# AIGC-Audio/AudioGPT

Hardware: AMD Instinct MI355X
Metric: generated audio-seconds/sec (10s clip, 100 DDIM steps) [3 independent batches of 8 prompts in flight per GPU] (higher is better)
Workload: dtype bf16x3; 1 GPU; Make-An-Audio T2A batch=8/GPU, 100 DDIM steps, CFG 1.5, UNet+VAE+HiFi-GAN(16k), fp32 storage, bf16x3-split MFMA (hi/lo, fp32 accumulate; meets the fp32 parity gates); prompts_per_gpu=8, ddim_steps=100, mel_frames=624, hipgraph=True, batches_in_flight=3, cfg_lanes=1, concurrency_hint=3, parallelism=prompt-sharded x1 (RCCL bcast cond / gather wav)

## Files before the change

### audiogpt_amd/_lib.py

```python
import ctypes as C
import os

import torch

_HERE = os.path.dirname(os.path.abspath(__file__))
LIB_PATH = os.environ.get("AUDIOGPT_AMD_LIB") or os.path.join(_HERE, "libaudiogpt_mi355x.so")


class MaaError(RuntimeError):
    pass


class maa_tensor(C.Structure):
    _fields_ = [("name", C.c_char_p), ("data", C.POINTER(C.c_float)), ("ndim", C.c_int), ("shape", C.c_int64 * 6)]


class maa_prof_row(C.Structure):
    _fields_ = [("name", C.c_char * 48), ("launches", C.c_int64), ("ms", C.c_double), ("flops", C.c_double),
                ("bytes", C.c_double)]


class maa_unet_config(C.Structure):
    _fields_ = [("in_channels", C.c_int), ("out_channels", C.c_int), ("model_channels", C.c_int),
                ("num_res_blocks", C.c_int),
# ... 22 lines not shown
                ("embed_dim", C.c_int), ("resolution", C.c_int), ("num_res_blocks", C.c_int), ("double_z", C.c_int),
                ("n_ch_mult", C.c_int), ("ch_mult", C.c_int * 8),
                ("n_attn_resolutions", C.c_int), ("attn_resolutions", C.c_int * 8)]


class maa_vocoder_config(C.Structure):
    _fields_ = [("kind", C.c_int), ("num_mels", C.c_int), ("upsample_initial_channel", C.c_int),
                ("n_upsamples", C.c_int), ("upsample_rates", C.c_int * 8), ("upsample_kernel_sizes", C.c_int * 8),
                ("n_kernels", C.c_int), ("resblock_kernel_sizes", C.c_int * 8),
                ("n_dilations", C.c_int), ("resblock_dilation_sizes", (C.c_int * 8) * 8),
                ("snake_beta", C.c_int), ("snake_logscale", C.c_int),
                ("use_pitch_embed", C.c_int), ("sampling_rate", C.c_int), ("harmonic_num", C.c_int),
                ("resblock", C.c_int)]


class maa_diffnet_config(C.Structure):
    _fields_ = [("in_dims", C.c_int), ("hidden_size", C.c_int), ("residual_layers", C.c_int),
                ("residual_channels", C.c_int), ("dilation_cycle_length", C.c_int)]


class maa_encoder_config(C.Structure):
    _fields_ = [("kind", C.c_int), ("layers", C.c_int), ("width", C.c_int), ("heads", C.c_int), ("mlp_dim", C.c_int),
                ("d_proj", C.c_int), ("vocab", C.c_int), ("max_positions", C.c_int), ("patch", C.c_int),
                ("image", C.c_int), ("ln_eps", C.c_float)]


class maa_clap_audio_config(C.Structure):
    _fields_ = [("mel_bins", C.c_int), ("n_blocks", C.c_int), ("channels", C.c_int * 8), ("out_emb", C.c_int),
                ("d_proj", C.c_int), ("bn_eps", C.c_float)]


class maa_spectral_config(C.Structure):
    _fields_ = [("n_fft", C.c_int), ("hop", C.c_int), ("n_freq", C.c_int), ("n_mels", C.c_int), ("pad_mode", C.c_int),
                ("power", C.c_int), ("log_kind", C.c_int), ("amin", C.c_float), ("ref", C.c_float), ("out_layout", C.c_int)]


class maa_plms_args(C.Structure):
    _fields_ = [("B", C.c_int), ("T", C.c_int), ("K_step", C.c_int), ("interval", C.c_int), ("timesteps", C.c_int),
                ("d_cond", C.c_void_p), ("h_alphas_cumprod", C.POINTER(C.c_float)), ("use_graph", C.c_int)]


EXPORTS = [
    "maa_last_error", "maa_version", "maa_ctx_create", "maa_ctx_destroy", "maa_ctx_synchronize",
    "maa_ctx_set_stream", "maa_ctx_set_precision", "maa_ctx_set_cfg_split", "maa_ctx_set_concurrency", "maa_ctx_reload_tuning", "maa_ctx_workspace_bytes", "maa_prof_begin", "maa_prof_end", "maa_unet_create", "maa_unet_destroy",
    "maa_unet_set_context", "maa_unet_forward", "maa_ddim_update", "maa_ddim_sample", "maa_ddim_stochastic_encode", "maa_ddim_decode",
    "maa_ldm_plms_sample",
    "maa_vae_create",
    "maa_vae_destroy", "maa_vae_decode", "maa_vae_decode_spec", "maa_vae_encode_moments", "maa_vocoder_create", "maa_vocoder_destroy",
    "maa_vocoder_forward", "maa_vocoder_forward_f0", "maa_diffnet_create", "maa_diffnet_destroy", "maa_diffnet_forward",
    "maa_plms_sample", "maa_encoder_create", "maa_encoder_destroy", "maa_encoder_text", "maa_encoder_image",
    "maa_encoder_text_cls", "maa_clap_audio_create", "maa_clap_audio_destroy", "maa_clap_audio_embed", "maa_clap_similarity",
    "maa_spectral_create", "maa_spectral_destroy", "maa_spectral_forward", "maa_resampler_create", "maa_resampler_destroy",
    "maa_resampler_forward", "maa_op_linear", "maa_op_conv", "maa_op_groupnorm", "maa_op_layernorm",
    "maa_op_attention", "maa_op_conv_transpose1d", "maa_op_snake_aa", "maa_op_bench_conv", "maa_calib",
]

_lib = None


def load():
    global _lib
    if _lib is not None:
        return _lib
    if not os.path.exists(LIB_PATH):
        raise MaaError("%s not found -- run `python -m audiogpt_amd.build` (hipcc, gfx950)" % LIB_PATH)
    try:
        lib = C.CDLL(LIB_PATH)
    except OSError as e:
        raise MaaError("cannot load %s: %s" % (LIB_PATH, e))
    vp, ci, cf, fp = C.c_void_p, C.c_int, C.c_float, C.POINTER(C.c_float)
    lib.maa_last_error.restype = C.c_char_p
    lib.maa_version.restype = C.c_char_p
    sig = {
        "maa_ctx_create": [ci, vp, C.POINTER(vp)],
        "maa_ctx_destroy": [vp],
        "maa_ctx_synchronize": [vp],
        "maa_ctx_set_stream": [vp, vp],
        "maa_ctx_workspace_bytes": [vp, C.POINTER(C.c_size_t)],
        "maa_ctx_set_precision": [vp, ci],
        "maa_ctx_set_cfg_split": [vp, ci],
        "maa_ctx_set_concurrency": [vp, ci],
        "maa_ctx_reload_tuning": [vp],
        "maa_prof_begin": [vp, ci],
        "maa_prof_end": [vp, C.POINTER(maa_prof_row), ci, C.POINTER(ci)],
        "maa_unet_create": [vp, C.POINTER(maa_unet_config), C.POINTER(maa_tensor), ci, C.POINTER(vp)],
        "maa_unet_destroy": [vp],
        "maa_unet_set_context": [vp, vp, vp, ci, ci],
        "maa_unet_forward": [vp, vp, vp, vp, ci, ci, ci, vp],
        "maa_ddim_update": [vp, vp, vp, vp, cf, vp, C.c_int64, vp, vp],
        "maa_ddim_sample": [vp, vp, C.POINTER(maa_ddim_args), vp],
        "maa_ddim_stochastic_encode": [vp, vp, ci, cf, vp, vp, fp, fp, ci, vp, ci, ci, ci, ci, vp],
        "maa_ddim_decode": [vp, vp, C.POINTER(maa_ddim_args), ci, vp],
        "maa_ldm_plms_sample": [vp, vp, C.POINTER(maa_ddim_args), vp],
        "maa_vae_create": [vp, C.POINTER(maa_vae_config), C.POINTER(maa_tensor), ci, C.POINTER(vp)],
        "maa_vae_destroy": [vp],
        "maa_vae_decode": [vp, vp, vp, ci, ci, ci, cf, vp],
        "maa_vae_decode_spec": [vp, vp, vp, ci, ci, ci, cf, vp],
        "maa_vae_encode_moments": [vp, vp, vp, ci, ci, ci, vp],
        "maa_vocoder_create": [vp, C.POINTER(maa_vocoder_config), C.POINTER(maa_tensor), ci, C.POINTER(vp)],
        "maa_vocoder_destroy": [vp],
        "maa_vocoder_forward": [vp, vp, vp, ci, ci, vp],
        "maa_vocoder_forward_f0": [vp, vp, vp, vp, vp, vp, ci, ci, vp],
        "maa_diffnet_create": [vp, C.POINTER(maa_diffnet_config), C.POINTER(maa_tensor), ci, C.POINTER(vp)],
        "maa_diffnet_destroy": [vp],
        "maa_diffnet_forward": [vp, vp, vp, vp, vp, ci, ci, vp],
        "maa_plms_sample": [vp, vp, C.POINTER(maa_plms_args), vp],
        "maa_encoder_create": [vp, C.POINTER(maa_encoder_config), C.POINTER(maa_tensor), ci, C.POINTER(vp)],
        "maa_encoder_destroy": [vp],
        "maa_encoder_text": [vp, vp, vp, ci, ci, vp],
        "maa_encoder_image": [vp, vp, vp, ci, vp],
        "maa_encoder_text_cls": [vp, vp, vp, ci, ci, vp],
        "maa_clap_audio_create": [vp, C.POINTER(maa_clap_audio_config), C.POINTER(maa_tensor), ci, C.POINTER(vp)],
        "maa_clap_audio_destroy": [vp],
        "maa_clap_audio_embed": [vp, vp, vp, ci, ci, vp, vp],
        "maa_clap_similarity": [vp, vp, vp, ci, ci, ci, cf, vp],
        "maa_spectral_create": [vp, C.POINTER(maa_spectral_config), fp, fp, C.POINTER(vp)],
        "maa_spectral_destroy": [vp],
        "maa_spectral_forward": [vp, vp, vp, ci, ci, vp],
        "maa_resampler_create": [vp, ci, ci, ci, ci, fp, C.POINTER(vp)],
        "maa_resampler_destroy": [vp],
        "maa_resampler_forward": [vp, vp, vp, ci, ci, vp],
        "maa_op_linear": [vp, vp, ci, ci, fp, fp, ci, ci, vp],
        "maa_op_conv": [vp, vp, ci, ci, ci, ci, fp, fp, ci, ci, ci, ci, ci, ci, ci, cf, vp, ci, ci],
        "maa_op_groupnorm": [vp, vp, ci, ci, ci, fp, fp, cf, ci, vp],
        "maa_op_layernorm": [vp, vp, ci, ci, fp, fp, cf, vp],
        "maa_op_attention": [vp, vp, vp, vp, ci, ci, ci, ci, ci, cf, vp],
        "maa_op_conv_transpose1d": [vp, vp, ci, ci, ci, fp, fp, ci, ci, ci, cf, vp],
        "maa_op_snake_aa": [vp, vp, ci, ci, ci, fp, fp, ci, vp],
        "maa_op_bench_conv": [vp, ci, ci, ci, ci, ci, ci, ci, ci, C.POINTER(C.c_float)],
        "maa_calib": [vp, ci, C.POINTER(C.c_double)],
    }
    for name, argtypes in sig.items():
        fn = getattr(lib, name)
        fn.argtypes = argtypes
        fn.restype = ci
    _lib = lib
    return lib


def check(status):
    if status != 0:
        raise MaaError("libaudiogpt_mi355x: %s (status %d)" % (load().maa_last_error().decode(), status))


def host_f32(t):
    t = t.detach().to(device="cpu", dtype=torch.float32).contiguous()
    return t, C.cast(t.data_ptr(), C.POINTER(C.c_float))


def tensor_list(state_dict):
    items = list(state_dict.items())
    arr = (maa_tensor * len(items))()
    keep = []
    for i, (name, t) in enumerate(items):
        ht, ptr = host_f32(t)
        bname = name.encode()
        keep.append((ht, bname))
        arr[i].name = bname
        arr[i].data = ptr
        arr[i].ndim = ht.dim()
        for d, s in enumerate(ht.shape):
            arr[i].shape[d] = s
    return arr, len(items), keep


def dptr(t):
    assert t.is_cuda and t.dtype == torch.float32 and t.is_contiguous(), (t.device, t.dtype, t.is_contiguous())
    return C.c_void_p(t.data_ptr())
```

### audiogpt_amd/backend.py

```python
import ctypes as C
import threading
import weakref

import numpy as np
import torch

from . import _lib as L


def default_precision():
    import os
    p = os.environ.get("AUDIOGPT_AMD_PRECISION", "bf16x3")
    if p not in Context.PRECISIONS:
        raise ValueError("AUDIOGPT_AMD_PRECISION must be one of %s" % sorted(Context.PRECISIONS))
    return p


_contexts = weakref.WeakSet()


def reload_tuning():
    for c in list(_contexts):
        c.reload_tuning()

# ... 73 lines not shown
    def __del__(self):
        try:
            self.close()
        except Exception:
            pass

    def op_linear(self, a, w, b=None, geglu=False):
        a = _f32(a, self.device)
        M, K = a.shape
        N = w.shape[0]
        wt, wp = L.host_f32(w)
        bt, bp = L.host_f32(b) if b is not None else (None, None)
        y = torch.empty(M, N // 2 if geglu else N, device=self.device)
        L.check(self.lib.maa_op_linear(self.h, L.dptr(a), M, K, wp, bp, N, int(geglu), L.dptr(y)))
        return y

    def op_conv(self, x, w, b=None, stride=1, pad=0, dil=1, up=False, leaky=0.0, out_hw=None):
        x = _f32(x, self.device)
        B, Cin, H, W = x.shape
        Cout, _, KH, KW = w.shape
        if out_hw is None:
            He, We = (2 * H, 2 * W) if up else (H, W)
            ph = pad if KH > 1 else 0
            Ho = (He + 2 * ph - dil * (KH - 1) - 1) // stride + 1
            Wo = (We + 2 * pad - dil * (KW - 1) - 1) // stride + 1
        else:
            Ho, Wo = out_hw
        wt, wp = L.host_f32(w)
        bt, bp = L.host_f32(b) if b is not None else (None, None)
        y = torch.empty(B, Cout, Ho, Wo, device=self.device)
        L.check(self.lib.maa_op_conv(self.h, L.dptr(x), B, Cin, H, W, wp, bp, Cout, KH, KW, stride, pad, dil,
                                     int(up), float(leaky), L.dptr(y), Ho, Wo))
        return y

    def op_groupnorm(self, x, gamma, beta, eps, silu=False):
        x = _f32(x, self.device)
        B, Cc = x.shape[:2]
        HW = int(np.prod(x.shape[2:]))
        gt, gp = L.host_f32(gamma)
        bt, bp = L.host_f32(beta)
        y = torch.empty_like(x)
        L.check(self.lib.maa_op_groupnorm(self.h, L.dptr(x), B, Cc, HW, gp, bp, float(eps), int(silu), L.dptr(y)))
        return y

    def op_layernorm(self, x, gamma, beta, eps=1e-5):
        x = _f32(x, self.device)
        rows, Cc = x.reshape(-1, x.shape[-1]).shape
        gt, gp = L.host_f32(gamma)
        bt, bp = L.host_f32(beta)
        y = torch.empty_like(x)
        L.check(self.lib.maa_op_layernorm(self.h, L.dptr(x), rows, Cc, gp, bp, float(eps), L.dptr(y)))
        return y

    def op_attention(self, q, k, v, heads, alpha):
        q, k, v = _f32(q, self.device), _f32(k, self.device), _f32(v, self.device)
        B, Nq, Cc = q.shape
        Nk = k.shape[1]
        y = torch.empty_like(q)
        L.check(self.lib.maa_op_attention(self.h, L.dptr(q), L.dptr(k), L.dptr(v), B, heads, Cc // heads, Nq, Nk,
                                          float(alpha), L.dptr(y)))
        return y

    def op_conv_transpose1d(self, x, w, b, stride, leaky=0.0):
        x = _f32(x, self.device)
        B, Cin, Ln = x.shape
        _, Cout, k = w.shape
        wt, wp = L.host_f32(w)
        bt, bp = L.host_f32(b)
        y = torch.empty(B, Cout, Ln * stride, device=self.device)
        L.check(self.lib.maa_op_conv_transpose1d(self.h, L.dptr(x), B, Cin, Ln, wp, bp, Cout, k, stride, float(leaky),
                                                 L.dptr(y)))
        return y

    def op_bench_conv(self, B, H, W, Cin, Cout, taps=9, pre_split=True, iters=20):
        ms = C.c_float()
        L.check(self.lib.maa_op_bench_conv(self.h, B, H, W, Cin, Cout, taps, int(pre_split), iters, C.byref(ms)))
        return ms.value

    def op_snake_aa(self, x, alpha, beta, logscale):
        x = _f32(x, self.device)
        B, Cc, Ln = x.shape
        at, ap = L.host_f32(alpha)
        bt, bp = L.host_f32(beta)
        y = torch.empty_like(x)
        L.check(self.lib.maa_op_snake_aa(self.h, L.dptr(x), B, Cc, Ln, ap, bp, int(logscale), L.dptr(y)))
        return y


def _fill(arr, values):
    for i, v in enumerate(values):
        arr[i] = int(v)
    return len(values)


class UNet:

    def __init__(self, ctx, cfg, state_dict):
        self.ctx, self.cfg = ctx, cfg
        c = L.maa_unet_config()
        c.in_channels, c.out_channels, c.model_channels = cfg["in_channels"], cfg["out_channels"], cfg["model_channels"]
        c.num_res_blocks = cfg["num_res_blocks"]
        c.n_channel_mult = _fill(c.channel_mult, cfg["channel_mult"])
        c.n_attention_resolutions = _fill(c.attention_resolutions, cfg["attention_resolutions"])
        c.num_heads, c.num_head_channels = cfg["num_heads"], cfg["num_head_channels"]
        c.use_spatial_transformer = int(cfg["use_spatial_transformer"])
        c.transformer_depth = cfg.get("transformer_depth", 1)
        c.context_dim = cfg["context_dim"] or 0
        c.legacy, c.resblock_updown = int(cfg["legacy"]), int(cfg["resblock_updown"])
        c.add_context_to_emb = int(cfg.get("add_context_to_emb", False))
        arr, n, keep = L.tensor_list(state_dict)
        h = C.c_void_p()
        with ctx.lock:
            L.check(ctx.lib.maa_unet_create(ctx.h, C.byref(c), arr, n, C.byref(h)))
# ... 625 lines not shown
```

### audiogpt_amd/csrc/api.cpp

```cpp
#include "models.h"

#include <cstring>
#include <memory>

namespace maa {
const char* last_error_cstr();
}

struct maa_ctx {
    maa::Ctx c;
    bool owns_stream = false;
};
struct maa_unet {
    std::unique_ptr<maa::UNet> m;
};
struct maa_vae {
    std::unique_ptr<maa::VAE> m;
};
struct maa_vocoder {
    std::unique_ptr<maa::Vocoder> m;
};
struct maa_diffnet {
    std::unique_ptr<maa::DiffNet> m;
};
// ... 605 lines not shown
    });
}

int maa_calib(maa_ctx* ctx, int kind, double* out_value) {
    return guarded([&] {
        bind(ctx);
        MAA_CHECK(out_value && kind >= 0 && kind <= 3, "bad calib arguments");
        *out_value = maa::calib_run(ctx->c, kind);
    });
}

int maa_op_groupnorm(maa_ctx* ctx, const float* d_x, int B, int C, int HW, const float* h_gamma, const float* h_beta,
                     float eps, int silu, float* d_y) {
    return guarded([&] {
        bind(ctx);
        MAA_CHECK(d_x && h_gamma && h_beta && d_y, "bad op_groupnorm arguments");
        maa::WeightStore ws(ctx->c.dtype != 0);
        maa::Ctx& c = ctx->c;
        float* g = ws.upload(std::vector<float>(h_gamma, h_gamma + C));
        float* b = ws.upload(std::vector<float>(h_beta, h_beta + C));
        maa::run_sized(c, [&] {
            maa::T4 x = maa::alloc_t(c, B, 1, HW, C), y = maa::alloc_t(c, B, 1, HW, C);
            maa::launch_nchw_to_nhwc(c, d_x, B, C, HW, x.p);
            maa::launch_groupnorm(c, x.p, C, C, nullptr, 0, 0, B, HW, 32, g, b, eps, silu, y.p);
            maa::launch_nhwc_to_nchw(c, y.p, B, C, HW, d_y, C);
        });
        MAA_HIP(hipStreamSynchronize(c.stream));
    });
}

int maa_op_layernorm(maa_ctx* ctx, const float* d_x, int rows, int C, const float* h_gamma, const float* h_beta,
                     float eps, float* d_y) {
    return guarded([&] {
        bind(ctx);
        MAA_CHECK(d_x && h_gamma && h_beta && d_y, "bad op_layernorm arguments");
        maa::WeightStore ws(ctx->c.dtype != 0);
        maa::Ctx& c = ctx->c;
        float* g = ws.upload(std::vector<float>(h_gamma, h_gamma + C));
        float* b = ws.upload(std::vector<float>(h_beta, h_beta + C));
        maa::launch_layernorm(c, d_x, rows, C, g, b, eps, d_y);
        MAA_HIP(hipStreamSynchronize(c.stream));
    });
}

int maa_op_attention(maa_ctx* ctx, const float* d_q, const float* d_k, const float* d_v, int B, int heads, int dh,
                     int Nq, int Nk, float alpha, float* d_y) {
    return guarded([&] {
        bind(ctx);
        MAA_CHECK(d_q && d_k && d_v && d_y, "bad op_attention arguments");
        maa::Ctx& c = ctx->c;
        const int C = heads * dh;
        maa::run_sized(c, [&] {
            maa::attention_into(c, d_q, C, dh, d_k, C, dh, d_v, C, dh, B, heads, dh, Nq, Nk, alpha, d_y, C);
        });
        MAA_HIP(hipStreamSynchronize(c.stream));
    });
}

int maa_op_conv_transpose1d(maa_ctx* ctx, const float* d_x, int B, int Cin, int L, const float* h_w,
                            const float* h_bias, int Cout, int k, int stride, float leaky_slope, float* d_y) {
    return guarded([&] {
        bind(ctx);
        MAA_CHECK(d_x && h_w && h_bias && d_y, "bad op_conv_transpose1d arguments");
        OneShot s;
        s.add("w", h_w, {Cin, Cout, k});
        s.add("b", h_bias, {Cout});
        maa::WeightStore ws(ctx->c.dtype != 0);
        maa::Ctx& c = ctx->c;
        const int pad = (k - stride) / 2, U = k / stride;
        maa::run_sized(c, [&] {
            maa::T4 x = maa::alloc_t(c, B, 1, L, Cin), y = maa::alloc_t(c, B, 1, L * stride, Cout);
            maa::launch_nchw_to_nhwc(c, d_x, B, Cin, L, x.p);
            for (int carry = 0; carry < 2; ++carry) {
                bool any = false;
                for (int r = 0; r < stride; ++r) any = any || ((r + pad) / stride == carry);
                if (!any) continue;
                int r_start = 0, r_count = 0;
                maa::PackedW pw;
                if (!c.ws.dry) pw = ws.pack_convtr_phase(s.sd, "w", "b", stride, pad, carry, &r_start, &r_count);
                maa::IGemm p;
                p.a1 = x.p;
                p.lda1 = Cin;
                p.C1 = Cin;
                p.Win = L;
                p.Wout = L;
                p.KW = U;
                p.pw = U - 1 - carry;
                if (leaky_slope != 0.f) {
                    p.a_act = 1;
                    p.a_slope = leaky_slope;
                }
                p.b = pw.w;
                p.ldb = pw.ld;
                p.b_nk = pw.nk;
                p.b_split = pw.split;
                p.M = B * L;
                p.K = U * Cin;
                p.N = r_count * Cout;
                p.bias = pw.bias;
                p.c = y.p + (long long)r_start * Cout;
                p.ldc = stride * Cout;
                if (!c.ws.dry) maa::launch_igemm(c, p);
            }
            maa::launch_nhwc_to_nchw(c, y.p, B, Cout, L * stride, d_y, Cout);
        });
        MAA_HIP(hipStreamSynchronize(c.stream));
// ... 114 lines not shown
```

### audiogpt_amd/csrc/flash_attn.hip

```cpp
#include "maa_internal.h"

#include <cstdlib>

namespace maa {

typedef float f32x16 __attribute__((ext_vector_type(16)));
typedef __bf16 bf16x8 __attribute__((ext_vector_type(8)));
typedef __bf16 bf16x2 __attribute__((ext_vector_type(2)));
typedef float f32x2 __attribute__((ext_vector_type(2)));

struct FlashArgs {
    const float *q, *k, *v;
    int ldq, ldk, ldv;
    int hsq, hsk, hsv;
    long long q_bs, k_bs, v_bs;
    int heads, Nq, Nk;
    float scale;
    float* out;
    int ldo;
    int out_split;
    int causal;
    int qtiles, xcd_on;
    long long o_bs;
    const float* zeros;
};

namespace {

constexpr int NT = 256;
constexpr int KT = 32;

__device__ __forceinline__ unsigned pk_bf16(float a, float b) {
    f32x2 f = {a, b};
    bf16x2 h = __builtin_convertvector(f, bf16x2);
    return __builtin_bit_cast(unsigned, h);
}
__device__ __forceinline__ void split2(float a, float b, unsigned& hi, unsigned& lo) {
    hi = pk_bf16(a, b);
    lo = pk_bf16(a - __builtin_bit_cast(float, hi << 16), b - __builtin_bit_cast(float, hi & 0xffff0000u));
}
struct Frag {
    unsigned w[4];
};
__device__ __forceinline__ bf16x8 as_bf16x8(const Frag& f) { return __builtin_bit_cast(bf16x8, f); }

template <int DH, int TERMS>
__global__ __launch_bounds__(NT, 1) void flash_attn_kernel(const FlashArgs a) {
    constexpr int DK = (DH + 15) / 16 * 16;
    constexpr int DM = (DH + 31) / 32 * 32;
    constexpr int KS = DK / 16, MB = DM / 32;
    constexpr int PL = TERMS == 1 ? 1 : 2;
    constexpr int LDKK = DK + 8;
    constexpr int LDV = KT + 4;
    constexpr int K_PLANE = KT * LDKK, V_PLANE = DM * LDV;
    constexpr int BUF = PL * (K_PLANE + V_PLANE);
    constexpr int C4 = DH / 4;
    static_assert(DH % 8 == 0, "head dim");
    extern __shared__ __attribute__((aligned(16))) unsigned short smem[];

    const int tid = threadIdx.x, lane = tid & 63, wid = tid >> 6;
    const int lq = lane & 31, lh = lane >> 5;
    const int w = xcd_contiguous((int)blockIdx.x, (int)gridDim.x, a.xcd_on);
    const int bh = w / a.qtiles, b = bh / a.heads, h = bh - b * a.heads;
    const int q0 = (w - bh * a.qtiles) * 128 + wid * 32;
    const bool wave_live = q0 < a.Nq;
    const float* qp = a.q + b * a.q_bs + h * a.hsq;
    const float* kp = a.k + b * a.k_bs + h * a.hsk;
    const float* vp = a.v + b * a.v_bs + h * a.hsv;
    const float4* zero4 = reinterpret_cast<const float4*>(a.zeros);

    for (int i = tid; i < 2 * BUF / 2; i += NT) reinterpret_cast<unsigned*>(smem)[i] = 0u;

    Frag qh[KS], ql[KS];
    {
        const int qrow = q0 + lq;
        const bool qok = qrow < a.Nq;
        const float* src = qp + (long long)(qok ? qrow : 0) * a.ldq;
        const float qs = a.scale * 1.4426950408889634f;
#pragma unroll
        for (int ks = 0; ks < KS; ++ks) {
            const int d = ks * 16 + lh * 8;
            float4 x0 = *((qok && d < DH) ? reinterpret_cast<const float4*>(src + d) : zero4);
            float4 x1 = *((qok && d + 4 < DH) ? reinterpret_cast<const float4*>(src + d + 4) : zero4);
            x0.x *= qs;
            x0.y *= qs;
            x0.z *= qs;
            x0.w *= qs;
            x1.x *= qs;
            x1.y *= qs;
            x1.z *= qs;
            x1.w *= qs;
            if constexpr (TERMS == 1) {
                qh[ks].w[0] = pk_bf16(x0.x, x0.y);
                qh[ks].w[1] = pk_bf16(x0.z, x0.w);
                qh[ks].w[2] = pk_bf16(x1.x, x1.y);
                qh[ks].w[3] = pk_bf16(x1.z, x1.w);
            } else {
                split2(x0.x, x0.y, qh[ks].w[0], ql[ks].w[0]);
                split2(x0.z, x0.w, qh[ks].w[1], ql[ks].w[1]);
                split2(x1.x, x1.y, qh[ks].w[2], ql[ks].w[2]);
                split2(x1.z, x1.w, qh[ks].w[3], ql[ks].w[3]);
            }
        }
    }

    constexpr int C2 = DH / 2;
    constexpr int NK = KT * C4, NV = (KT / 4) * C2;
    constexpr int NLK = (NK + NT - 1) / NT, NLV = (NV + NT - 1) / NT;
    float4 rk[NLK];
    float2 rv[NLV][4];
    const float2* zero2 = reinterpret_cast<const float2*>(a.zeros);
    auto load_tile = [&](int kt) {
#pragma unroll
        for (int j = 0; j < NLK; ++j) {
            const int idx = tid + NT * j;
            const int key = idx / C4, c4 = idx - key * C4;
            const int kg = kt * KT + key;
            const bool ok = idx < NK && kg < a.Nk;
            rk[j] = *(ok ? reinterpret_cast<const float4*>(kp + (long long)kg * a.ldk + c4 * 4) : zero4);
        }
#pragma unroll
        for (int j = 0; j < NLV; ++j) {
            const int idx = (NT - 1 - tid) + NT * j;
            const int kb = idx / C2, c2 = idx - kb * C2;
#pragma unroll
            for (int k = 0; k < 4; ++k) {
                const int kg = kt * KT + kb * 4 + k;
                const bool ok = idx < NV && kg < a.Nk;
                rv[j][k] = *(ok ? reinterpret_cast<const float2*>(vp + (long long)kg * a.ldv + c2 * 2) : zero2);
            }
        }
    };
    auto store_tile = [&](int buf) {
        unsigned short* base = smem + buf * BUF;
        unsigned short* vt = base + PL * K_PLANE;
#pragma unroll
        for (int j = 0; j < NLK; ++j) {
            const int idx = tid + NT * j;
            if (idx < NK) {
                const int key = idx / C4, c4 = idx - key * C4;
                uint2 hi, lo;
                if constexpr (TERMS == 1) {
                    hi.x = pk_bf16(rk[j].x, rk[j].y);
                    hi.y = pk_bf16(rk[j].z, rk[j].w);
                } else {
                    split2(rk[j].x, rk[j].y, hi.x, lo.x);
                    split2(rk[j].z, rk[j].w, hi.y, lo.y);
                    *reinterpret_cast<uint2*>(base + K_PLANE + key * LDKK + c4 * 4) = lo;
                }
                *reinterpret_cast<uint2*>(base + key * LDKK + c4 * 4) = hi;
            }
        }
#pragma unroll
        for (int j = 0; j < NLV; ++j) {
            const int idx = (NT - 1 - tid) + NT * j;
            if (idx < NV) {
                const int kb = idx / C2, c2 = idx - kb * C2;
                auto put = [&](int d, float v0, float v1, float v2, float v3) {
                    uint2 hi, lo;
                    if constexpr (TERMS == 1) {
                        hi.x = pk_bf16(v0, v1);
                        hi.y = pk_bf16(v2, v3);
                    } else {
                        split2(v0, v1, hi.x, lo.x);
                        split2(v2, v3, hi.y, lo.y);
                        *reinterpret_cast<uint2*>(vt + V_PLANE + d * LDV + kb * 4) = lo;
                    }
                    *reinterpret_cast<uint2*>(vt + d * LDV + kb * 4) = hi;
                };
                put(2 * c2, rv[j][0].x, rv[j][1].x, rv[j][2].x, rv[j][3].x);
                put(2 * c2 + 1, rv[j][0].y, rv[j][1].y, rv[j][2].y, rv[j][3].y);
            }
        }
    };

    f32x16 oacc[MB];
#pragma unroll
    for (int mb = 0; mb < MB; ++mb)
#pragma unroll
        for (int r = 0; r < 16; ++r) oacc[mb][r] = 0.f;
    float m_run = -INFINITY, l_run = 0.f;

    const int ntiles = (a.Nk + KT - 1) / KT;
    load_tile(0);
    __syncthreads();
    store_tile(0);
    __syncthreads();

    for (int kt = 0; kt < ntiles; ++kt) {
        const int buf = kt & 1;
        load_tile(kt + 1);
        const unsigned short* base = smem + buf * BUF;
        const unsigned short* vt = base + PL * K_PLANE;

        if (wave_live) {
            f32x16 sacc;
    #pragma unroll
            for (int r = 0; r < 16; ++r) sacc[r] = 0.f;
    #pragma unroll
            for (int ks = 0; ks < KS; ++ks) {
                const bf16x8 kh = *reinterpret_cast<const bf16x8*>(base + lq * LDKK + ks * 16 + lh * 8);
                if constexpr (TERMS == 3) {
                    const bf16x8 kl = *reinterpret_cast<const bf16x8*>(base + K_PLANE + lq * LDKK + ks * 16 + lh * 8);
                    sacc = __builtin_amdgcn_mfma_f32_32x32x16_bf16(kl, as_bf16x8(qh[ks]), sacc, 0, 0, 0);
                    sacc = __builtin_amdgcn_mfma_f32_32x32x16_bf16(kh, as_bf16x8(ql[ks]), sacc, 0, 0, 0);
                }
                sacc = __builtin_amdgcn_mfma_f32_32x32x16_bf16(kh, as_bf16x8(qh[ks]), sacc, 0, 0, 0);
            }

            float p[16];
            float mt = -INFINITY;
            if (!a.causal && (kt + 1) * KT <= a.Nk) {
    #pragma unroll
                for (int r = 0; r < 16; ++r) {
                    p[r] = sacc[r];
                    mt = fmaxf(mt, p[r]);
                }
            } else {
    #pragma unroll
                for (int r = 0; r < 16; ++r) {
                    const int key = kt * KT + (r & 3) + 8 * (r >> 2) + 4 * lh;
                    p[r] = (key < a.Nk && (!a.causal || key <= q0 + lq)) ? sacc[r] : -INFINITY;
                    mt = fmaxf(mt, p[r]);
                }
            }
            mt = fmaxf(mt, __shfl_xor(mt, 32, 64));
            const float m_new = fmaxf(m_run, mt);
            float alpha, ls = 0.f;
            alpha = __builtin_amdgcn_exp2f(m_run - m_new);
    #pragma unroll
            for (int r = 0; r < 16; ++r) {
                p[r] = __builtin_amdgcn_exp2f(p[r] - m_new);
                ls += p[r];
            }
            ls += __shfl_xor(ls, 32, 64);
            l_run = l_run * alpha + ls;
            const bool moved = m_new != m_run;
            m_run = m_new;
            if (__any(moved)) {
    #pragma unroll
                for (int mb = 0; mb < MB; ++mb)
    #pragma unroll
                    for (int r = 0; r < 16; ++r) oacc[mb][r] *= alpha;
            }

    #pragma unroll
            for (int u = 0; u < 2; ++u) {
                Frag ph, pl;
    #pragma unroll
                for (int t = 0; t < 4; ++t) {
                    if constexpr (TERMS == 1)
                        ph.w[t] = pk_bf16(p[8 * u + 2 * t], p[8 * u + 2 * t + 1]);
                    else
                        split2(p[8 * u + 2 * t], p[8 * u + 2 * t + 1], ph.w[t], pl.w[t]);
                }
    #pragma unroll
                for (int mb = 0; mb < MB; ++mb) {
                    const unsigned short* vrow = vt + (mb * 32 + lq) * LDV + 16 * u + 4 * lh;
                    Frag vh, vl;
                    const uint2 a0 = *reinterpret_cast<const uint2*>(vrow);
                    const uint2 a1 = *reinterpret_cast<const uint2*>(vrow + 8);
                    vh.w[0] = a0.x;
                    vh.w[1] = a0.y;
                    vh.w[2] = a1.x;
                    vh.w[3] = a1.y;
                    if constexpr (TERMS == 3) {
                        const uint2 c0 = *reinterpret_cast<const uint2*>(vrow + V_PLANE);
                        const uint2 c1 = *reinterpret_cast<const uint2*>(vrow + V_PLANE + 8);
                        vl.w[0] = c0.x;
                        vl.w[1] = c0.y;
                        vl.w[2] = c1.x;
                        vl.w[3] = c1.y;
                        oacc[mb] = __builtin_amdgcn_mfma_f32_32x32x16_bf16(as_bf16x8(vl), as_bf16x8(ph), oacc[mb], 0, 0, 0);
                        oacc[mb] = __builtin_amdgcn_mfma_f32_32x32x16_bf16(as_bf16x8(vh), as_bf16x8(pl), oacc[mb], 0, 0, 0);
                    }
                    oacc[mb] = __builtin_amdgcn_mfma_f32_32x32x16_bf16(as_bf16x8(vh), as_bf16x8(ph), oacc[mb], 0, 0, 0);
                }
            }

        }
        store_tile(buf ^ 1);
        __syncthreads();
    }

    float* ot = reinterpret_cast<float*>(smem) + wid * 32 * (DM + 1);
    const float inv = 1.f / l_run;
#pragma unroll
    for (int mb = 0; mb < MB; ++mb)
#pragma unroll
        for (int r = 0; r < 16; ++r) {
            const int d = mb * 32 + (r & 3) + 8 * (r >> 2) + 4 * lh;
            ot[lq * (DM + 1) + d] = oacc[mb][r] * inv;
        }
    __syncthreads();
    float* op = a.out + b * a.o_bs + h * DH;
    if (a.out_split) {
        for (int i = lane; i < 16 * DH; i += 64) {
            const int qi = i / (DH / 2), d = (i - qi * (DH / 2)) * 2;
            if (q0 + qi < a.Nq) {
                const float v0 = ot[qi * (DM + 1) + d], v1 = ot[qi * (DM + 1) + d + 1];
                unsigned hi, lo;
                split2(v0, v1, hi, lo);
                const int c = h * DH + d;
                unsigned short* o = reinterpret_cast<unsigned short*>(a.out + b * a.o_bs + (long long)(q0 + qi) * a.ldo) +
                                    (c >> 5) * 64 + (c & 31);
                *reinterpret_cast<unsigned*>(o) = hi;
                *reinterpret_cast<unsigned*>(o + 32) = lo;
            }
        }
    } else {
        for (int i = lane; i < 32 * DH; i += 64) {
            const int qi = i / DH, d = i - qi * DH;
            if (q0 + qi < a.Nq) op[(long long)(q0 + qi) * a.ldo + d] = ot[qi * (DM + 1) + d];
        }
    }
}

template <int DH, int TERMS>
void launch_dh(const Ctx& ctx, const FlashArgs& a, int B) {
    constexpr int DK = (DH + 15) / 16 * 16, DM = (DH + 31) / 32 * 32, PL = TERMS == 1 ? 1 : 2;
    constexpr size_t kv = (size_t)2 * PL * (KT * (DK + 8) + DM * (KT + 4)) * sizeof(unsigned short);
    constexpr size_t tr = (size_t)4 * 32 * (DM + 1) * sizeof(float);
    constexpr size_t lds = kv > tr ? kv : tr;
    auto kern = flash_attn_kernel<DH, TERMS>;
    ensure_dynamic_lds(reinterpret_cast<const void*>(kern), ctx.device, (int)lds);
    dim3 grid((unsigned)(a.qtiles * B * a.heads));
    hipLaunchKernelGGL(kern, grid, dim3(NT), lds, ctx.stream, a);
}

}

bool flash_attention_covers(const Ctx& ctx, int dh) {
    return ctx.dtype != 0 && (dh == 32 || dh == 40 || dh == 64 || dh == 80);
}

bool launch_flash_attention(const Ctx& ctx, const float* q, int ldq, int hsq, const float* k, int ldk, int hsk,
                            const float* v, int ldv, int hsv, int B, int heads, int dh, int Nq, int Nk, float alpha,
                            float* out, int ldo, int out_split, int causal) {
    if (!flash_attention_covers(ctx, dh)) return false;
    auto al16 = [](const void* p) { return (reinterpret_cast<uintptr_t>(p) & 15) == 0; };
    if (ldq % 4 || ldk % 4 || ldv % 4 || hsq % 4 || hsk % 4 || hsv % 4 || !al16(q) || !al16(k) || !al16(v)) return false;
    if (ctx.ws.dry) return true;
    FlashArgs a;
    a.q = q;
    a.k = k;
    a.v = v;
    a.ldq = ldq;
    a.ldk = ldk;
    a.ldv = ldv;
    a.hsq = hsq;
    a.hsk = hsk;
    a.hsv = hsv;
    a.q_bs = (long long)Nq * ldq;
    a.k_bs = (long long)Nk * ldk;
    a.v_bs = (long long)Nk * ldv;
    a.heads = heads;
    a.Nq = Nq;
    a.Nk = Nk;
    a.scale = alpha;
    a.out = out;
    a.ldo = ldo;
    a.out_split = out_split;
    a.causal = causal;
    a.o_bs = (long long)Nq * ldo;
    a.zeros = ctx.zeros;
    a.qtiles = (Nq + 127) / 128;
    a.xcd_on = 1;
    const double flops = 4.0 * B * heads * (double)Nq * Nk * dh;
    const double bytes = 4.0 * B * heads * ((double)2 * Nq * dh + 2.0 * Nk * dh);
    ProfScope prof(ctx, "flash_attention", flops, bytes);
    const int terms = ctx.dtype == 1 ? 3 : 1;
#define MAA_FLASH(DHV)                                 \
    if (terms == 3)                                    \
        launch_dh<DHV, 3>(ctx, a, B);                  \
    else                                               \
        launch_dh<DHV, 1>(ctx, a, B);
// ... 13 lines not shown
```

### include/maa.h

```cpp
#ifndef MAA_H_
#define MAA_H_

#include <stddef.h>
#include <stdint.h>

#ifdef __cplusplus
extern "C" {
#endif

typedef enum maa_status {
    MAA_OK = 0,
    MAA_ERR_INVALID = -1,
    MAA_ERR_HIP = -2,
    MAA_ERR_INTERNAL = -3
} maa_status;

typedef struct maa_ctx maa_ctx;
typedef struct maa_unet maa_unet;
typedef struct maa_vae maa_vae;
typedef struct maa_vocoder maa_vocoder;

const char* maa_last_error(void);
const char* maa_version(void);

// ... 135 lines not shown
                       maa_encoder** out);
int maa_encoder_destroy(maa_encoder* e);
int maa_encoder_text(maa_ctx* ctx, maa_encoder* e, const int* d_ids, int B, int L, float* d_out);
int maa_encoder_image(maa_ctx* ctx, maa_encoder* e, const float* d_img, int B, float* d_out);

int maa_encoder_text_cls(maa_ctx* ctx, maa_encoder* e, const int* d_ids, int B, int L, float* d_out);

typedef struct maa_clap_audio_config {
    int mel_bins, n_blocks, channels[8];
    int out_emb, d_proj;
    float bn_eps;
} maa_clap_audio_config;
typedef struct maa_clap_audio maa_clap_audio;
int maa_clap_audio_create(maa_ctx* ctx, const maa_clap_audio_config* cfg, const maa_tensor* tensors, int n_tensors,
                          maa_clap_audio** out);
int maa_clap_audio_destroy(maa_clap_audio* a);
int maa_clap_audio_embed(maa_ctx* ctx, maa_clap_audio* a, const float* d_logmel, int B, int T, float* d_embedding,
                         float* d_z);
int maa_clap_similarity(maa_ctx* ctx, const float* d_audio, const float* d_text, int Na, int Nt, int D, float scale,
                        float* d_out);

typedef struct maa_spectral_config {
    int n_fft, hop, n_freq, n_mels;
    int pad_mode;
    int power;
    int log_kind;
    float amin, ref;
    int out_layout;
} maa_spectral_config;
typedef struct maa_spectral maa_spectral;
int maa_spectral_create(maa_ctx* ctx, const maa_spectral_config* cfg, const float* h_basis, const float* h_melw,
                        maa_spectral** out);
int maa_spectral_destroy(maa_spectral* s);
int maa_spectral_forward(maa_ctx* ctx, maa_spectral* s, const float* d_wav, int B, int n, float* d_out);

typedef struct maa_resampler maa_resampler;
int maa_resampler_create(maa_ctx* ctx, int orig, int neu, int width, int klen, const float* h_kernels, maa_resampler** out);
int maa_resampler_destroy(maa_resampler* r);
int maa_resampler_forward(maa_ctx* ctx, maa_resampler* r, const float* d_wav, int B, int n, float* d_out);

int maa_calib(maa_ctx* ctx, int kind, double* out_value);

int maa_op_linear(maa_ctx* ctx, const float* d_a, int M, int K, const float* h_w, const float* h_bias, int N,
                  int geglu, float* d_y);
int maa_op_conv(maa_ctx* ctx, const float* d_x, int B, int Cin, int H, int W, const float* h_w, const float* h_bias,
                int Cout, int KH, int KW, int stride, int pad, int dil, int upsample2, float leaky_slope,
                float* d_y, int Ho, int Wo);
int maa_op_groupnorm(maa_ctx* ctx, const float* d_x, int B, int C, int HW, const float* h_gamma,
                     const float* h_beta, float eps, int silu, float* d_y);
int maa_op_layernorm(maa_ctx* ctx, const float* d_x, int rows, int C, const float* h_gamma, const float* h_beta,
                     float eps, float* d_y);
int maa_op_attention(maa_ctx* ctx, const float* d_q, const float* d_k, const float* d_v, int B, int heads, int dh,
                     int Nq, int Nk, float alpha, float* d_y);
int maa_op_conv_transpose1d(maa_ctx* ctx, const float* d_x, int B, int Cin, int L, const float* h_w,
                            const float* h_bias, int Cout, int k, int stride, float leaky_slope, float* d_y);
int maa_op_bench_conv(maa_ctx* ctx, int B, int H, int W, int Cin, int Cout, int taps, int pre_split, int iters,
                      float* ms_per_launch);
int maa_op_snake_aa(maa_ctx* ctx, const float* d_x, int B, int C, int L, const float* h_alpha, const float* h_beta,
                    int logscale, float* d_y);

#ifdef __cplusplus
}
#endif
#endif
```

Baseline: 136.0 audio-seconds/sec.

## Restructure flash attention: split K/V pipeline, prefetch QK, 16x16 PV MFMA

Reworks the flash attention kernel so K and V tiles are staged separately, with K prefetched two tiles ahead. The QK^T for the next tile is computed while softmax and PV run on the current tile, overlapping MFMA work with the exp/reduction phase. PV now uses 16x16x32 MFMAs fed by permlane swaps, which removes padding to 32 in the head dimension (e.g. dh=40/80) and drops the LDS transpose in the epilogue by writing outputs straight from registers. It also adds an attention_ex op entry with out_split/causal flags, at the cost of more registers and more complex lane mapping.

```diff
diff --git a/audiogpt_amd/_lib.py b/audiogpt_amd/_lib.py
--- a/audiogpt_amd/_lib.py
+++ b/audiogpt_amd/_lib.py
@@ -98,7 +98,7 @@
     "maa_encoder_text_cls", "maa_clap_audio_create", "maa_clap_audio_destroy", "maa_clap_audio_embed", "maa_clap_similarity",
     "maa_spectral_create", "maa_spectral_destroy", "maa_spectral_forward", "maa_resampler_create", "maa_resampler_destroy",
     "maa_resampler_forward", "maa_op_linear", "maa_op_conv", "maa_op_groupnorm", "maa_op_layernorm",
-    "maa_op_attention", "maa_op_conv_transpose1d", "maa_op_snake_aa", "maa_op_bench_conv", "maa_calib",
+    "maa_op_attention", "maa_op_attention_ex", "maa_op_conv_transpose1d", "maa_op_snake_aa", "maa_op_bench_conv", "maa_calib",
 ]
 
 _lib = None
@@ -171,6 +171,7 @@
         "maa_op_groupnorm": [vp, vp, ci, ci, ci, fp, fp, cf, ci, vp],
         "maa_op_layernorm": [vp, vp, ci, ci, fp, fp, cf, vp],
         "maa_op_attention": [vp, vp, vp, vp, ci, ci, ci, ci, ci, cf, vp],
+        "maa_op_attention_ex": [vp, vp, vp, vp, ci, ci, ci, ci, ci, cf, ci, ci, vp],
         "maa_op_conv_transpose1d": [vp, vp, ci, ci, ci, fp, fp, ci, ci, ci, cf, vp],
         "maa_op_snake_aa": [vp, vp, ci, ci, ci, fp, fp, ci, vp],
         "maa_op_bench_conv": [vp, ci, ci, ci, ci, ci, ci, ci, ci, C.POINTER(C.c_float)],
diff --git a/audiogpt_amd/backend.py b/audiogpt_amd/backend.py
--- a/audiogpt_amd/backend.py
+++ b/audiogpt_amd/backend.py
@@ -149,13 +149,17 @@
         L.check(self.lib.maa_op_layernorm(self.h, L.dptr(x), rows, Cc, gp, bp, float(eps), L.dptr(y)))
         return y
 
-    def op_attention(self, q, k, v, heads, alpha):
+    def op_attention(self, q, k, v, heads, alpha, out_split=False, causal=False):
         q, k, v = _f32(q, self.device), _f32(k, self.device), _f32(v, self.device)
         B, Nq, Cc = q.shape
         Nk = k.shape[1]
         y = torch.empty_like(q)
-        L.check(self.lib.maa_op_attention(self.h, L.dptr(q), L.dptr(k), L.dptr(v), B, heads, Cc // heads, Nq, Nk,
-                                          float(alpha), L.dptr(y)))
+        if out_split or causal:
+            L.check(self.lib.maa_op_attention_ex(self.h, L.dptr(q), L.dptr(k), L.dptr(v), B, heads, Cc // heads, Nq, Nk,
+                                                 float(alpha), int(out_split), int(causal), L.dptr(y)))
+        else:
+            L.check(self.lib.maa_op_attention(self.h, L.dptr(q), L.dptr(k), L.dptr(v), B, heads, Cc // heads, Nq, Nk,
+                                              float(alpha), L.dptr(y)))
         return y
 
     def op_conv_transpose1d(self, x, w, b, stride, leaky=0.0):
diff --git a/audiogpt_amd/csrc/api.cpp b/audiogpt_amd/csrc/api.cpp
--- a/audiogpt_amd/csrc/api.cpp
+++ b/audiogpt_amd/csrc/api.cpp
@@ -681,6 +681,21 @@
         const int C = heads * dh;
         maa::run_sized(c, [&] {
             maa::attention_into(c, d_q, C, dh, d_k, C, dh, d_v, C, dh, B, heads, dh, Nq, Nk, alpha, d_y, C);
+        });
+        MAA_HIP(hipStreamSynchronize(c.stream));
+    });
+}
+
+int maa_op_attention_ex(maa_ctx* ctx, const float* d_q, const float* d_k, const float* d_v, int B, int heads, int dh,
+                        int Nq, int Nk, float alpha, int out_split, int causal, float* d_y) {
+    return guarded([&] {
+        bind(ctx);
+        MAA_CHECK(d_q && d_k && d_v && d_y, "bad op_attention arguments");
+        maa::Ctx& c = ctx->c;
+        const int C = heads * dh;
+        maa::run_sized(c, [&] {
+            maa::attention_into(c, d_q, C, dh, d_k, C, dh, d_v, C, dh, B, heads, dh, Nq, Nk, alpha, d_y, C, out_split ? 1 : 0,
+                                causal ? 1 : 0);
         });
         MAA_HIP(hipStreamSynchronize(c.stream));
     });
diff --git a/audiogpt_amd/csrc/flash_attn.hip b/audiogpt_amd/csrc/flash_attn.hip
--- a/audiogpt_amd/csrc/flash_attn.hip
+++ b/audiogpt_amd/csrc/flash_attn.hip
@@ -5,6 +5,7 @@
 namespace maa {
 
 typedef float f32x16 __attribute__((ext_vector_type(16)));
+typedef float f32x4 __attribute__((ext_vector_type(4)));
 typedef __bf16 bf16x8 __attribute__((ext_vector_type(8)));
 typedef __bf16 bf16x2 __attribute__((ext_vector_type(2)));
 typedef float f32x2 __attribute__((ext_vector_type(2)));
@@ -43,23 +44,40 @@
     unsigned w[4];
 };
 __device__ __forceinline__ bf16x8 as_bf16x8(const Frag& f) { return __builtin_bit_cast(bf16x8, f); }
+__device__ __forceinline__ float pairmax(float x) {
+    const auto r = __builtin_amdgcn_permlane32_swap(__float_as_uint(x), __float_as_uint(x), false, false);
+    return fmaxf(__uint_as_float(r[0]), __uint_as_float(r[1]));
+}
+__device__ __forceinline__ float pairsum(float x) {
+    const auto r = __builtin_amdgcn_permlane32_swap(__float_as_uint(x), __float_as_uint(x), false, false);
+    return __uint_as_float(r[0]) + __uint_as_float(r[1]);
+}
+__device__ __forceinline__ void qblocks(float x, float& x0, float& x1) {
+    const auto r = __builtin_amdgcn_permlane16_swap(__float_as_uint(x), __float_as_uint(x), false, false);
+    x0 = __uint_as_float(r[0]);
+    x1 = __uint_as_float(r[1]);
+}
 
 template <int DH, int TERMS>
 __global__ __launch_bounds__(NT, 1) void flash_attn_kernel(const FlashArgs a) {
     constexpr int DK = (DH + 15) / 16 * 16;
-    constexpr int DM = (DH + 31) / 32 * 32;
-    constexpr int KS = DK / 16, MB = DM / 32;
+    constexpr int KS = DK / 16;
+    constexpr int DB = (DH + 15) / 16;
+    constexpr int DM = DB * 16;
     constexpr int PL = TERMS == 1 ? 1 : 2;
     constexpr int LDKK = DK + 8;
-    constexpr int LDV = KT + 4;
+    constexpr int LDV = KT + 8;
     constexpr int K_PLANE = KT * LDKK, V_PLANE = DM * LDV;
-    constexpr int BUF = PL * (K_PLANE + V_PLANE);
+    constexpr int KBUF = PL * K_PLANE, VBUF = PL * V_PLANE;
     constexpr int C4 = DH / 4;
     static_assert(DH % 8 == 0, "head dim");
     extern __shared__ __attribute__((aligned(16))) unsigned short smem[];
+    unsigned short* const kbufs = smem;
+    unsigned short* const vbufs = smem + 2 * KBUF;
 
     const int tid = threadIdx.x, lane = tid & 63, wid = tid >> 6;
     const int lq = lane & 31, lh = lane >> 5;
+    const int l16 = lane & 15, lg = lane >> 4;
     const int w = xcd_contiguous((int)blockIdx.x, (int)gridDim.x, a.xcd_on);
     const int bh = w / a.qtiles, b = bh / a.heads, h = bh - b * a.heads;
     const int q0 = (w - bh * a.qtiles) * 128 + wid * 32;
@@ -69,7 +87,7 @@
     const float* vp = a.v + b * a.v_bs + h * a.hsv;
     const float4* zero4 = reinterpret_cast<const float4*>(a.zeros);
 
-    for (int i = tid; i < 2 * BUF / 2; i += NT) reinterpret_cast<unsigned*>(smem)[i] = 0u;
+    for (int i = tid; i < (2 * KBUF + 2 * VBUF) / 2; i += NT) reinterpret_cast<unsigned*>(smem)[i] = 0u;
 
     Frag qh[KS], ql[KS];
     {
@@ -110,7 +128,7 @@
     float4 rk[NLK];
     float2 rv[NLV][4];
     const float2* zero2 = reinterpret_cast<const float2*>(a.zeros);
-    auto load_tile = [&](int kt) {
+    auto load_k = [&](int kt) {
 #pragma unroll
         for (int j = 0; j < NLK; ++j) {
             const int idx = tid + NT * j;
@@ -119,6 +137,8 @@
             const bool ok = idx < NK && kg < a.Nk;
             rk[j] = *(ok ? reinterpret_cast<const float4*>(kp + (long long)kg * a.ldk + c4 * 4) : zero4);
         }
+    };
+    auto load_v = [&](int kt) {
 #pragma unroll
         for (int j = 0; j < NLV; ++j) {
             const int idx = (NT - 1 - tid) + NT * j;
@@ -131,9 +151,8 @@
             }
         }
     };
-    auto store_tile = [&](int buf) {
-        unsigned short* base = smem + buf * BUF;
-        unsigned short* vt = base + PL * K_PLANE;
+    auto store_k = [&](int buf) {
+        unsigned short* base = kbufs + buf * KBUF;
 #pragma unroll
         for (int j = 0; j < NLK; ++j) {
             const int idx = tid + NT * j;
@@ -151,11 +170,15 @@
                 *reinterpret_cast<uint2*>(base + key * LDKK + c4 * 4) = hi;
             }
         }
+    };
+    auto store_v = [&](int buf) {
+        unsigned short* vt = vbufs + buf * VBUF;
 #pragma unroll
         for (int j = 0; j < NLV; ++j) {
             const int idx = (NT - 1 - tid) + NT * j;
             if (idx < NV) {
                 const int kb = idx / C2, c2 = idx - kb * C2;
+                const int col = 4 * ((kb >> 1) + 4 * (kb & 1));
                 auto put = [&](int d, float v0, float v1, float v2, float v3) {
                     uint2 hi, lo;
                     if constexpr (TERMS == 1) {
@@ -164,9 +187,9 @@
                     } else {
                         split2(v0, v1, hi.x, lo.x);
                         split2(v2, v3, hi.y, lo.y);
-                        *reinterpret_cast<uint2*>(vt + V_PLANE + d * LDV + kb * 4) = lo;
+                        *reinterpret_cast<uint2*>(vt + V_PLANE + d * LDV + col) = lo;
                     }
-                    *reinterpret_cast<uint2*>(vt + d * LDV + kb * 4) = hi;
+                    *reinterpret_cast<uint2*>(vt + d * LDV + col) = hi;
                 };
                 put(2 * c2, rv[j][0].x, rv[j][1].x, rv[j][2].x, rv[j][3].x);
                 put(2 * c2 + 1, rv[j][0].y, rv[j][1].y, rv[j][2].y, rv[j][3].y);
@@ -174,154 +197,165 @@
         }
     };
 
-    f32x16 oacc[MB];
-#pragma unroll
-    for (int mb = 0; mb < MB; ++mb)
-#pragma unroll
-        for (int r = 0; r < 16; ++r) oacc[mb][r] = 0.f;
+    auto qk = [&](const unsigned short* base) {
+        f32x16 s;
+#pragma unroll
+        for (int r = 0; r < 16; ++r) s[r] = 0.f;
+#pragma unroll
+        for (int ks = 0; ks < KS; ++ks) {
+            const bf16x8 kh = *reinterpret_cast<const bf16x8*>(base + lq * LDKK + ks * 16 + lh * 8);
+            if constexpr (TERMS == 3) {
+                const bf16x8 kl = *reinterpret_cast<const bf16x8*>(base + K_PLANE + lq * LDKK + ks * 16 + lh * 8);
+                s = __builtin_amdgcn_mfma_f32_32x32x16_bf16(kl, as_bf16x8(qh[ks]), s, 0, 0, 0);
+                s = __builtin_amdgcn_mfma_f32_32x32x16_bf16(kh, as_bf16x8(ql[ks]), s, 0, 0, 0);
+            }
+            s = __builtin_amdgcn_mfma_f32_32x32x16_bf16(kh, as_bf16x8(qh[ks]), s, 0, 0, 0);
+        }
+        return s;
+    };
+
+    f32x4 o0[DB], o1[DB];
+#pragma unroll
+    for (int db = 0; db < DB; ++db)
+#pragma unroll
+        for (int i = 0; i < 4; ++i) {
+            o0[db][i] = 0.f;
+            o1[db][i] = 0.f;
+        }
     float m_run = -INFINITY, l_run = 0.f;
 
     const int ntiles = (a.Nk + KT - 1) / KT;
-    load_tile(0);
+    load_k(0);
+    load_v(0);
     __syncthreads();
-    store_tile(0);
+    store_k(0);
+    store_v(0);
+    load_k(1);
     __syncthreads();
+    f32x16 s_cur = {};
+    if (wave_live) s_cur = qk(kbufs);
+    store_k(1);
+    __syncthreads();
 
     for (int kt = 0; kt < ntiles; ++kt) {
-        const int buf = kt & 1;
-        load_tile(kt + 1);
-        const unsigned short* base = smem + buf * BUF;
-        const unsigned short* vt = base + PL * K_PLANE;
+        load_k(kt + 2);
+        load_v(kt + 1);
 
         if (wave_live) {
-            f32x16 sacc;
-    #pragma unroll
-            for (int r = 0; r < 16; ++r) sacc[r] = 0.f;
-    #pragma unroll
-            for (int ks = 0; ks < KS; ++ks) {
-                const bf16x8 kh = *reinterpret_cast<const bf16x8*>(base + lq * LDKK + ks * 16 + lh * 8);
-                if constexpr (TERMS == 3) {
-                    const bf16x8 kl = *reinterpret_cast<const bf16x8*>(base + K_PLANE + lq * LDKK + ks * 16 + lh * 8);
-                    sacc = __builtin_amdgcn_mfma_f32_32x32x16_bf16(kl, as_bf16x8(qh[ks]), sacc, 0, 0, 0);
-                    sacc = __builtin_amdgcn_mfma_f32_32x32x16_bf16(kh, as_bf16x8(ql[ks]), sacc, 0, 0, 0);
-                }
-                sacc = __builtin_amdgcn_mfma_f32_32x32x16_bf16(kh, as_bf16x8(qh[ks]), sacc, 0, 0, 0);
-            }
-
             float p[16];
-            float mt = -INFINITY;
             if (!a.causal && (kt + 1) * KT <= a.Nk) {
-    #pragma unroll
-                for (int r = 0; r < 16; ++r) {
-                    p[r] = sacc[r];
-                    mt = fmaxf(mt, p[r]);
-                }
+#pragma unroll
+                for (int r = 0; r < 16; ++r) p[r] = s_cur[r];
             } else {
-    #pragma unroll
+#pragma unroll
                 for (int r = 0; r < 16; ++r) {
                     const int key = kt * KT + (r & 3) + 8 * (r >> 2) + 4 * lh;
-                    p[r] = (key < a.Nk && (!a.causal || key <= q0 + lq)) ? sacc[r] : -INFINITY;
-                    mt = fmaxf(mt, p[r]);
+                    p[r] = (key < a.Nk && (!a.causal || key <= q0 + lq)) ? s_cur[r] : -INFINITY;
                 }
             }
-            mt = fmaxf(mt, __shfl_xor(mt, 32, 64));
-            const float m_new = fmaxf(m_run, mt);
-            float alpha, ls = 0.f;
-            alpha = __builtin_amdgcn_exp2f(m_run - m_new);
-    #pragma unroll
+            const f32x16 s_next = qk(kbufs + ((kt + 1) & 1) * KBUF);
+
+            float mt = p[0];
+#pragma unroll
+            for (int r = 1; r < 16; ++r) mt = fmaxf(mt, p[r]);
+            const float m_new = fmaxf(m_run, pairmax(mt));
+            const float alpha = __builtin_amdgcn_exp2f(m_run - m_new);
+            float ls = 0.f;
+#pragma unroll
             for (int r = 0; r < 16; ++r) {
                 p[r] = __builtin_amdgcn_exp2f(p[r] - m_new);
                 ls += p[r];
             }
-            ls += __shfl_xor(ls, 32, 64);
-            l_run = l_run * alpha + ls;
-            const bool moved = m_new != m_run;
+            l_run = l_run * alpha + pairsum(ls);
             m_run = m_new;
-            if (__any(moved)) {
-    #pragma unroll
-                for (int mb = 0; mb < MB; ++mb)
-    #pragma unroll
-                    for (int r = 0; r < 16; ++r) oacc[mb][r] *= alpha;
-            }
-
-    #pragma unroll
-            for (int u = 0; u < 2; ++u) {
-                Frag ph, pl;
-    #pragma unroll
+
+            Frag b0h, b1h, b0l, b1l;
+            {
+                unsigned ph[8], pl[8];
+#pragma unroll
+                for (int t = 0; t < 8; ++t) {
+                    if constexpr (TERMS == 1)
+                        ph[t] = pk_bf16(p[2 * t], p[2 * t + 1]);
+                    else
+                        split2(p[2 * t], p[2 * t + 1], ph[t], pl[t]);
+                }
+#pragma unroll
                 for (int t = 0; t < 4; ++t) {
-                    if constexpr (TERMS == 1)
-                        ph.w[t] = pk_bf16(p[8 * u + 2 * t], p[8 * u + 2 * t + 1]);
-                    else
-                        split2(p[8 * u + 2 * t], p[8 * u + 2 * t + 1], ph.w[t], pl.w[t]);
+                    const auto rh = __builtin_amdgcn_permlane16_swap(ph[t], ph[t + 4], false, false);
+                    b0h.w[t] = rh[0];
+                    b1h.w[t] = rh[1];
+                    if constexpr (TERMS == 3) {
+                        const auto rl = __builtin_amdgcn_permlane16_swap(pl[t], pl[t + 4], false, false);
+                        b0l.w[t] = rl[0];
+                        b1l.w[t] = rl[1];
+                    }
                 }
-    #pragma unroll
-                for (int mb = 0; mb < MB; ++mb) {
-                    const unsigned short* vrow = vt + (mb * 32 + lq) * LDV + 16 * u + 4 * lh;
-                    Frag vh, vl;
-                    const uint2 a0 = *reinterpret_cast<const uint2*>(vrow);
-                    const uint2 a1 = *reinterpret_cast<const uint2*>(vrow + 8);
-                    vh.w[0] = a0.x;
-                    vh.w[1] = a0.y;
-                    vh.w[2] = a1.x;
-                    vh.w[3] = a1.y;
-                    if constexpr (TERMS == 3) {
-                        const uint2 c0 = *reinterpret_cast<const uint2*>(vrow + V_PLANE);
-                        const uint2 c1 = *reinterpret_cast<const uint2*>(vrow + V_PLANE + 8);
-                        vl.w[0] = c0.x;
-                        vl.w[1] = c0.y;
-                        vl.w[2] = c1.x;
-                        vl.w[3] = c1.y;
-                        oacc[mb] = __builtin_amdgcn_mfma_f32_32x32x16_bf16(as_bf16x8(vl), as_bf16x8(ph), oacc[mb], 0, 0, 0);
-                        oacc[mb] = __builtin_amdgcn_mfma_f32_32x32x16_bf16(as_bf16x8(vh), as_bf16x8(pl), oacc[mb], 0, 0, 0);
-                    }
-                    oacc[mb] = __builtin_amdgcn_mfma_f32_32x32x16_bf16(as_bf16x8(vh), as_bf16x8(ph), oacc[mb], 0, 0, 0);
+            }
+            float a0, a1;
+            qblocks(alpha, a0, a1);
+
+            const unsigned short* vt = vbufs + (kt & 1) * VBUF + l16 * LDV + 8 * lg;
+#pragma unroll
+            for (int db = 0; db < DB; ++db) {
+                o0[db] *= a0;
+                o1[db] *= a1;
+                const bf16x8 vh = *reinterpret_cast<const bf16x8*>(vt + db * 16 * LDV);
+                if constexpr (TERMS == 3) {
+                    const bf16x8 vl = *reinterpret_cast<const bf16x8*>(vt + V_PLANE + db * 16 * LDV);
+                    o0[db] = __builtin_amdgcn_mfma_f32_16x16x32_bf16(vl, as_bf16x8(b0h), o0[db], 0, 0, 0);
+                    o0[db] = __builtin_amdgcn_mfma_f32_16x16x32_bf16(vh, as_bf16x8(b0l), o0[db], 0, 0, 0);
+                    o1[db] = __builtin_amdgcn_mfma_f32_16x16x32_bf16(vl, as_bf16x8(b1h), o1[db], 0, 0, 0);
+                    o1[db] = __builtin_amdgcn_mfma_f32_16x16x32_bf16(vh, as_bf16x8(b1l), o1[db], 0, 0, 0);
                 }
-            }
-
-        }
-        store_tile(buf ^ 1);
+                o0[db] = __builtin_amdgcn_mfma_f32_16x16x32_bf16(vh, as_bf16x8(b0h), o0[db], 0, 0, 0);
+                o1[db] = __builtin_amdgcn_mfma_f32_16x16x32_bf16(vh, as_bf16x8(b1h), o1[db], 0, 0, 0);
+            }
+            s_cur = s_next;
+        }
+        store_k(kt & 1);
+        store_v((kt + 1) & 1);
         __syncthreads();
     }
 
-    float* ot = reinterpret_cast<float*>(smem) + wid * 32 * (DM + 1);
-    const float inv = 1.f / l_run;
-#pragma unroll
-    for (int mb = 0; mb < MB; ++mb)
-#pragma unroll
-        for (int r = 0; r < 16; ++r) {
-            const int d = mb * 32 + (r & 3) + 8 * (r >> 2) + 4 * lh;
-            ot[lq * (DM + 1) + d] = oacc[mb][r] * inv;
-        }
-    __syncthreads();
-    float* op = a.out + b * a.o_bs + h * DH;
-    if (a.out_split) {
-        for (int i = lane; i < 16 * DH; i += 64) {
-            const int qi = i / (DH / 2), d = (i - qi * (DH / 2)) * 2;
-            if (q0 + qi < a.Nq) {
-                const float v0 = ot[qi * (DM + 1) + d], v1 = ot[qi * (DM + 1) + d + 1];
-                unsigned hi, lo;
-                split2(v0, v1, hi, lo);
+    float inv0, inv1;
+    qblocks(1.f / l_run, inv0, inv1);
+    float* ob = a.out + b * a.o_bs;
+#pragma unroll
+    for (int j = 0; j < 2; ++j) {
+        const int q = q0 + 16 * j + l16;
+        if (q >= a.Nq) continue;
+        const float inv = j ? inv1 : inv0;
+#pragma unroll
+        for (int db = 0; db < DB; ++db) {
+            const int d = 16 * db + 4 * lg;
+            if (d >= DH) continue;
+            const f32x4 o = (j ? o1[db] : o0[db]) * inv;
+            if (a.out_split) {
                 const int c = h * DH + d;
-                unsigned short* o = reinterpret_cast<unsigned short*>(a.out + b * a.o_bs + (long long)(q0 + qi) * a.ldo) +
-                                    (c >> 5) * 64 + (c & 31);
-                *reinterpret_cast<unsigned*>(o) = hi;
-                *reinterpret_cast<unsigned*>(o + 32) = lo;
-            }
-        }
-    } else {
-        for (int i = lane; i < 32 * DH; i += 64) {
-            const int qi = i / DH, d = i - qi * DH;
-            if (q0 + qi < a.Nq) op[(long long)(q0 + qi) * a.ldo + d] = ot[qi * (DM + 1) + d];
+                unsigned* os = reinterpret_cast<unsigned*>(reinterpret_cast<unsigned short*>(ob + (long long)q * a.ldo) +
+                                                           (c >> 5) * 64 + (c & 31));
+                unsigned h0, h1, e0, e1;
+                split2(o[0], o[1], h0, e0);
+                split2(o[2], o[3], h1, e1);
+                os[0] = h0;
+                os[1] = h1;
+                os[16] = e0;
+                os[17] = e1;
+            } else {
+                float* op = ob + (long long)q * a.ldo + h * DH + d;
+                op[0] = o[0];
+                op[1] = o[1];
+                op[2] = o[2];
+                op[3] = o[3];
+            }
         }
     }
 }
 
 template <int DH, int TERMS>
 void launch_dh(const Ctx& ctx, const FlashArgs& a, int B) {
-    constexpr int DK = (DH + 15) / 16 * 16, DM = (DH + 31) / 32 * 32, PL = TERMS == 1 ? 1 : 2;
-    constexpr size_t kv = (size_t)2 * PL * (KT * (DK + 8) + DM * (KT + 4)) * sizeof(unsigned short);
-    constexpr size_t tr = (size_t)4 * 32 * (DM + 1) * sizeof(float);
-    constexpr size_t lds = kv > tr ? kv : tr;
+    constexpr int DK = (DH + 15) / 16 * 16, DM = (DH + 15) / 16 * 16, PL = TERMS == 1 ? 1 : 2;
+    constexpr size_t lds = (size_t)2 * PL * (KT * (DK + 8) + DM * (KT + 8)) * sizeof(unsigned short);
     auto kern = flash_attn_kernel<DH, TERMS>;
     ensure_dynamic_lds(reinterpret_cast<const void*>(kern), ctx.device, (int)lds);
     dim3 grid((unsigned)(a.qtiles * B * a.heads));
diff --git a/include/maa.h b/include/maa.h
--- a/include/maa.h
+++ b/include/maa.h
@@ -211,6 +211,8 @@
                      float eps, float* d_y);
 int maa_op_attention(maa_ctx* ctx, const float* d_q, const float* d_k, const float* d_v, int B, int heads, int dh,
                      int Nq, int Nk, float alpha, float* d_y);
+int maa_op_attention_ex(maa_ctx* ctx, const float* d_q, const float* d_k, const float* d_v, int B, int heads, int dh,
+                        int Nq, int Nk, float alpha, int out_split, int causal, float* d_y);
 int maa_op_conv_transpose1d(maa_ctx* ctx, const float* d_x, int B, int Cin, int L, const float* h_w,
                             const float* h_bias, int Cout, int k, int stride, float leaky_slope, float* d_y);
 int maa_op_bench_conv(maa_ctx* ctx, int B, int H, int W, int Cin, int Cout, int taps, int pre_split, int iters,
```

Measured after the change: 136.4 audio-seconds/sec, median of 6. About the same (+0.3%).
